# Ushio/MassiveVoxelRayTracing

Measured on AMD Instinct MI355X. Metric: Mrays/sec (primary+secondary) at 1920x1080, 64 spp, higher is better.
Workload: dtype f32; 1 GPU; xyzrgb_dragon stand-in 2048^3 SVO (procedural, pinned by tests/test_scenes.py), wavefront path trace 1920x1080, 183 steps of 16 spp rendered as 64-spp frames (frame buffer cleared + device synchronised per frame), 8 bounces + IBL shadow rays; voxels=18903401, dag_nodes=643656, triangles=1102122, parallelism=1 GPU, device= (gfx950:sramecc+:xnack-, 256 CUs)

## Files before the change

massivevoxelraytracing_amd/csrc/api.hip:

```cpp
#include <stdarg.h>
#include <stdio.h>
#include <stdlib.h>
#include <string.h>

#include <string>
#include <utility>
#include <vector>

#include "../../include/mvrt.h"
#include "launch.h"
#include "traverse_stream.h"

#define MVRT_EXPORT extern "C" __attribute__( ( visibility( "default" ) ) )

static thread_local char g_err[1024] = "";
void mvrtSetError( const char* fmt, ... )
{
	va_list ap;
	va_start( ap, fmt );
	vsnprintf( g_err, sizeof( g_err ), fmt, ap );
	va_end( ap );
}
MVRT_EXPORT const char* mvrt_last_error( void ) { return g_err; }

// ... 1083 lines not shown
	REQUIRE( pt && pt->pmj.p && tableHost, "mvrt_pt_download_pmj: call mvrt_pt_setup first" );
	MVRT_HIP( hipMemcpy( tableHost, pt->pmj.p, pt->pmj.bytes, hipMemcpyDeviceToHost ) );
	return 0;
}

MVRT_EXPORT int mvrt_pt_set_tile( mvrt_pt* pt, int tileIndex, int tileCount )
{
	REQUIRE( pt && tileCount >= 1 && tileIndex >= 0 && tileIndex < tileCount, "bad tile %d of %d", tileIndex, tileCount );
	if( pt->drain() ) return 1;
	pt->tileIndex = tileIndex;
	pt->tileCount = tileCount;
	pt->width = pt->height = 0;
	pt->fbF32.release();
	pt->releaseAovs();
	pt->releaseMoments();
	return 0;
}
MVRT_EXPORT uint64_t mvrt_pt_owned_pixels( const mvrt_pt* pt ) { return pt ? pt->ownedPixels : 0; }

static int allocWorkSlot( mvrt_pt* pt, mvrt_pt::Slot& sl )
{
	const uint64_t cap = pt->ownedPixels * MVRT_SPP_PER_STEP * pt->effectiveBatch();
	const uint64_t nBlocks = cap / 256 + 8;
	const uint64_t words = cap * ( 34 + 6 + 1 + 3 + 4 );
	const uint64_t bytes = words * 4 + cap * 3 + nBlocks * 4 + 64 * 4 + 32 * 8 + 1024 + 64 * 256;
	if( sl.work.alloc( bytes ) ) return 1;
	uint8_t* base = (uint8_t*)sl.work.p;
	uint64_t off = 0;
	auto take = [&]( uint64_t b ) {
		void* r = base + off;
		off += ( b + 255 ) & ~(uint64_t)255;
		return r;
	};
	PtBuffers& b = sl.buf;
	for( int s = 0; s < 2; s++ )
	{
		PathSet& ps = b.set[s];
		ps.task = (uint32_t*)take( cap * 4 );
		ps.org = (uint32_t*)take( cap * 4 );
		float** f[] = { &ps.rox, &ps.roy, &ps.roz, &ps.rdx, &ps.rdy, &ps.rdz, &ps.Tx, &ps.Ty, &ps.Tz, &ps.Lx, &ps.Ly, &ps.Lz, &ps.nx, &ps.ny, &ps.nz };
		for( float** q : f ) *q = (float*)take( cap * 4 );
	}
	float** d[] = { &b.sx, &b.sy, &b.sz, &b.ex, &b.ey, &b.ez, &b.hitT, &b.Lsx, &b.Lsy, &b.Lsz };
	for( float** q : d ) *q = (float*)take( cap * 4 );
	b.hitPath = (uint64_t*)take( cap * 8 );
	b.hitEPath = (uint64_t*)take( cap * 8 );
	b.hitN = (uint8_t*)take( cap );
	b.hitS = (uint8_t*)take( cap );
	b.hitE = (uint8_t*)take( cap );
	b.blockCount = (uint32_t*)take( nBlocks * 4 );
	b.liveCount = (uint32_t*)take( 64 * 4 );
	b.cursors = (unsigned long long*)take( 16 * 8 );
	b.stats = pt->statsBuf.as<unsigned long long>();
	b.cap = cap;
	b.selfDev = (const PtBuffers*)take( sizeof( PtBuffers ) );
	MVRT_HIP( hipMemset( b.liveCount, 0, 64 * 4 ) );
	MVRT_HIP( hipMemcpy( (void*)b.selfDev, &b, sizeof( PtBuffers ), hipMemcpyHostToDevice ) );
	if( pt->aovs )
	{
		if( sl.aovPart.alloc( cap / MVRT_SPP_PER_STEP * 2 * sizeof( float4 ) ) ) return 1;
	}
	else sl.aovPart.release();
	return 0;
}
static int allocWorkInner( mvrt_pt* pt );
static int forgetFrame( mvrt_pt* pt )
{
	for( mvrt_pt::Slot& sl : pt->slots )
	{
		sl.work.release();
		memset( &sl.buf, 0, sizeof( sl.buf ) );
	}
	pt->width = pt->height = 0;
	pt->fbF32.release();
	pt->fbU8.release();
	pt->releaseAovs();
	pt->releaseMoments();
	return 1;
}
static int allocWork( mvrt_pt* pt ) { return allocWorkInner( pt ) == 0 ? 0 : forgetFrame( pt ); }
static int allocWorkInner( mvrt_pt* pt )
{
	if( pt->drain() ) return 1;
	if( !pt->statsBuf.p )
	{
		if( pt->statsBuf.alloc( 64 * 8 ) ) return 1;
		MVRT_HIP( hipMemset( pt->statsBuf.p, 0, 64 * 8 ) );
	}
	if( !pt->forkEv ) MVRT_HIP( hipEventCreateWithFlags( &pt->forkEv, hipEventDisableTiming ) );
	{
		for( mvrt_pt::Slot& sl : pt->slots )
		{
			sl.work.release();
			sl.aovPart.release();
			memset( &sl.buf, 0, sizeof( sl.buf ) );
		}
		size_t freeB = 0, totalB = 0;
		MVRT_HIP( hipMemGetInfo( &freeB, &totalB ) );
		if( pt->testFreeBytes ) freeB = (size_t)pt->testFreeBytes;
		pt->batchCap = MVRT_MAX_BATCH;
		pt->depth = pt->depthWanted;
		const uint64_t budget = (uint64_t)( 0.7 * (double)freeB );
		auto need = [&]() {
			const uint64_t pathState = (uint64_t)pt->depth * pt->ownedPixels * MVRT_SPP_PER_STEP * (uint64_t)pt->effectiveBatch() * 200ull;
			const uint64_t withAovs = pt->aovs ? pathState + (uint64_t)pt->depth * pt->ownedPixels * (uint64_t)pt->effectiveBatch() * 32ull + pt->ownedPixels * 32ull : pathState;
			return pt->moments ? withAovs + pt->ownedPixels * 16ull : withAovs;
		};
		while( need() > budget && pt->effectiveBatch() > 1 ) pt->batchCap = pt->effectiveBatch() - 1;
		while( need() > budget && pt->depth > 1 ) pt->depth--;
		REQUIRE( need() <= budget, "frame of %llu owned pixels needs %.1f GB of path state, %.1f GB of HBM are free (split the frame into tiles: mvrt_pt_set_tile)",
				 (unsigned long long)pt->ownedPixels, need() / 1e9, freeB / 1e9 );
	}
	for( int i = 0; i < 4; i++ )
	{
		mvrt_pt::Slot& sl = pt->slots[i];
		if( i >= pt->depth )
		{
			sl.work.release();
			sl.aovPart.release();
			sl.trace = Workspace();
			memset( &sl.buf, 0, sizeof( sl.buf ) );
			continue;
		}
		if( allocWorkSlot( pt, sl ) ) return 1;
		if( pt->depth > 1 && !sl.stream )
		{
			const int mode = (int)mvrtKnob( "MVRT_SLOT_PRIO", 0 );
// ... 631 lines not shown
```

massivevoxelraytracing_amd/csrc/kernels_rt.hip:

```cpp
#include <stdlib.h>

#include "launch.h"
#include "traverse_stream.h"

#define WAVE 64
#define CBLOCK 256

MVRT_DI uint32_t laneId() { return __builtin_amdgcn_mbcnt_hi( ~0u, __builtin_amdgcn_mbcnt_lo( ~0u, 0u ) ); }

MVRT_DI unsigned long long waveSum( unsigned long long v )
{
	for( int o = 32; o > 0; o >>= 1 ) v += __shfl_down( v, o, WAVE );
	return v;
}

static int numCUs();

#define STREAM_WAVES_PER_CU 32

struct BatchIO
{
	const float *rox, *roy, *roz, *rdx, *rdy, *rdz;
	const uint8_t* isShadow;
	float* tOut;
	int32_t* nMajorOut;
	uint64_t* pathOut;
	uint32_t* descentsOut;
#ifdef MVRT_UTIL_STATS
	unsigned long long utilIters = 0, utilActive = 0, utilTailIters = 0, utilTailActive = 0, utilRefillClocks = 0, utilTotalClocks = 0;
	uint32_t utilMaxRayIters = 0;
#endif
	const uint64_t* originPath;
	uint32_t levels;
	MVRT_DI bool load( uint32_t i, f3* ro, f3* rd, uint32_t* hint ) const
	{
		*ro = mk3( rox[i], roy[i], roz[i] );
		*rd = mk3( rdx[i], rdy[i], rdz[i] );
		if( originPath )
		{
			const uint64_t op = originPath[i];
			if( op != ~0ull ) *hint = hintFromVoxelPath( op, levels );
		}
		return isShadow ? isShadow[i] != 0 : false;
	}
	MVRT_DI void store( uint32_t i, const StreamHit& h, bool ) const
	{
		tOut[i] = h.t;
		if( nMajorOut ) nMajorOut[i] = h.nMajor;
		if( pathOut ) pathOut[i] = h.path;
		if( descentsOut ) descentsOut[i] = h.descents;
	}
};
__global__ void __launch_bounds__( 256 ) kResolveVIndex( SvoDev svo, uint64_t n, const float* __restrict__ t, const uint64_t* __restrict__ path, const uint8_t* __restrict__ isShadow,
														  uint32_t* __restrict__ vIndexOut, uchar4* __restrict__ colorOut )
{
	for( uint64_t i = (uint64_t)blockIdx.x * 256 + threadIdx.x; i < n; i += (uint64_t)gridDim.x * 256 )
// ... 19 lines not shown
template <int FL>
__global__ void __launch_bounds__( 64, MVRT_WAVES_OF( FL ) ) kTraceBatchStream( SvoDev svo, uint64_t n, BatchIO io, TraceWorkspace ws, uint32_t chunk )
{
	__shared__ uint4 ring[MVRT_RING_OF( FL ) * 64];
	__shared__ uint32_t ringMask[FL == 0 ? 1 : ( FL == 2 ? 2 : 1 ) * MVRT_RING_OF( FL ) * 64];
	traceStream<FL>( makeTraceCore( svo ), io, n, ws.cursor, chunk, ring, ws.spill, ws.spillStride, (uint64_t)blockIdx.x * 64 + threadIdx.x, ringMask, ws.spillMask, ws.spillMask2 );
}

struct PrimaryIO
{
	SvoDev svo;
	CameraPinhole cam;
	int W, H, showVertexColor;
	uchar4* rgba;
	float* tOut;
	int32_t* nMajorOut;
	uint64_t* pathOut;
	uint32_t* descentsOut;
#ifdef MVRT_UTIL_STATS
	unsigned long long utilIters = 0, utilActive = 0, utilTailIters = 0, utilTailActive = 0, utilRefillClocks = 0, utilTotalClocks = 0;
	uint32_t utilMaxRayIters = 0;
#endif
	f3 rdKeep;
	MVRT_DI bool load( uint32_t pixelIdx, f3* ro, f3* rd, uint32_t* )
	{
		int x = (int)( pixelIdx % W );
		int y = (int)( pixelIdx / W );
		cameraShoot( cam, ro, rd, x, y, 0.5f, 0.5f, W, H );
		rdKeep = *rd;
		return false;
	}
	MVRT_DI void store( uint32_t pixelIdx, const StreamHit& r, bool ) const
	{
		uchar4 c = make_uchar4( 0, 0, 0, 255 );
		if( r.t != MVRT_MAXF )
		{
			if( !showVertexColor )
			{
				f3 hn = getHitN( r.nMajor, rdKeep );
				f3 color = ( hn + mk3( 1.0f, 1.0f, 1.0f ) ) * 0.5f;
				c = make_uchar4( (uint8_t)( 255 * color.x + 0.5f ), (uint8_t)( 255 * color.y + 0.5f ), (uint8_t)( 255 * color.z + 0.5f ), 255 );
			}
		}
		if( rgba ) rgba[pixelIdx] = c;
		if( tOut ) tOut[pixelIdx] = r.t;
		if( nMajorOut ) nMajorOut[pixelIdx] = r.nMajor;
// ... 273 lines not shown
	*step = ps / vp;
	*localPixel = ps - *step * vp;
}

MVRT_DI int dimBase( int k, int hdriEnabled, int extraSamples ) { return 2 + k * ( ( hdriEnabled ? 2 : 0 ) + 1 ) + ( k > 0 ? extraSamples : 0 ); }

__global__ void __launch_bounds__( 256 ) kPtGenerate( PtParams P )
{
	const uint64_t n = P.frame.validOwnedPixels * MVRT_SPP_PER_STEP * P.frame.nSteps;
	const PathSet& o = P.buf.set[0];
	for( uint64_t task = (uint64_t)blockIdx.x * 256 + threadIdx.x; task < n; task += (uint64_t)gridDim.x * 256 )
	{
		uint32_t step, localPixel, localSpp;
		decodeTask( P.frame, (uint32_t)task, &step, &localPixel, &localSpp );
		uint32_t pixelIdx = globalPixel( P.frame, localPixel );
		int x = pixelIdx % P.frame.width;
		int y = pixelIdx / P.frame.width;
		uint32_t spp = ( P.frame.iteration + step ) * MVRT_SPP_PER_STEP + localSpp;
		uint32_t stream = hashCombine2( 0u, pixelIdx );
		f2 camU = pmjSample2d( P.pmj, spp, 0, stream );
		f2 lensU = pmjSample2d( P.pmj, spp, 1, stream );
		f3 ro, rd;
		cameraShootThinLens( P.cams[step], &ro, &rd, x, y, camU.x, camU.y, P.frame.width, P.frame.height, lensU.x, lensU.y );
		o.task[task] = (uint32_t)task;
		o.rox[task] = ro.x;
		o.roy[task] = ro.y;
		o.roz[task] = ro.z;
		o.rdx[task] = rd.x;
		o.rdy[task] = rd.y;
		o.rdz[task] = rd.z;
	}
	for( uint64_t b = (uint64_t)blockIdx.x * 256 + threadIdx.x; b < ( n + CBLOCK - 1 ) / CBLOCK; b += (uint64_t)gridDim.x * 256 ) P.buf.blockCount[b] = 0u;
	if( blockIdx.x == 0 && threadIdx.x == 0 )
	{
		P.buf.liveCount[0] = (uint32_t)n;
		for( int k = 0; k < 16; k++ ) P.buf.cursors[k] = 0ull;
		atomicAdd( &P.buf.stats[5], (unsigned long long)n );
	}
}

template <class T>
MVRT_DI const __attribute__( ( address_space( 4 ) ) ) T* opaquePtr( const T* p )
{
	asm volatile( "" : "+s"( p ) );
	return (const __attribute__( ( address_space( 4 ) ) ) T*)p;
}

struct PtIO
{
	const PtBuffers* table;
	int setIdx;
	uint32_t n;
	int shadowKind;
	int useHint;
#ifdef MVRT_UTIL_STATS
	unsigned long long utilIters = 0, utilActive = 0, utilTailIters = 0, utilTailActive = 0, utilRefillClocks = 0, utilTotalClocks = 0;
	uint32_t utilMaxRayIters = 0;
#endif
	uint32_t dNormal, dShadow, nHits;
	MVRT_DI int kindOf( uint32_t r, uint32_t* i ) const
	{
		const uint32_t kindSlot = ( r >= n ? 1u : 0u ) + ( r >= 2u * n ? 1u : 0u );
		*i = r - ( kindSlot == 0u ? 0u : ( kindSlot == 1u ? n : 2u * n ) );
		return kindSlot == 0 ? 0 : ( kindSlot == 1 ? ( shadowKind ? 1 : 2 ) : 2 );
	}
	MVRT_DI bool load( uint32_t r, f3* ro, f3* rd, uint32_t* hint ) const
	{
		const __attribute__( ( address_space( 4 ) ) ) PtBuffers& buf = *opaquePtr( table );
		const __attribute__( ( address_space( 4 ) ) ) PathSet& in = buf.set[setIdx];
		uint32_t i;
		const int kind = kindOf( r, &i );
		*ro = mk3( in.rox[i], in.roy[i], in.roz[i] );
		if( useHint ) *hint = in.org[i];
		if( kind == 0 ) *rd = mk3( in.rdx[i], in.rdy[i], in.rdz[i] );
		else if( kind == 1 ) *rd = mk3( buf.sx[i], buf.sy[i], buf.sz[i] );
		else *rd = mk3( buf.ex[i], buf.ey[i], buf.ez[i] );
		return kind == 1;
	}
	MVRT_DI void store( uint32_t r, const StreamHit& h, bool )
	{
		const __attribute__( ( address_space( 4 ) ) ) PtBuffers& buf = *opaquePtr( table );
		uint32_t i;
		const int kind = kindOf( r, &i );
		const bool isHit = h.t != MVRT_MAXF;
		if( kind == 0 )
		{
			buf.hitT[i] = h.t;
			buf.hitPath[i] = h.path;
			buf.hitN[i] = (uint8_t)h.nMajor;
			if( isHit ) atomicAdd( &buf.blockCount[i / CBLOCK], 1u );
		}
		else if( kind == 1 )
		{
			buf.hitS[i] = isHit ? 1 : 0;
		}
		else
		{
			buf.hitE[i] = isHit ? 1 : 0;
			buf.hitEPath[i] = h.path;
		}
		dShadow += kind == 1 ? h.descents : 0u;
		dNormal += kind == 1 ? 0u : h.descents;
		nHits += ( kind != 1 && isHit ) ? 1u : 0u;
	}
};
template <int FL>
__global__ void __launch_bounds__( 64, MVRT_WAVES_OF( FL ) ) kPtTraceStream( PtParams P, TraceWorkspace ws, int stage, int setIdx, int nKinds, int shadowKind, uint32_t chunk,
																			uint32_t raysPerLane, uint32_t minWaves )
{
	__shared__ uint4 ring[MVRT_RING_OF( FL ) * 64];
	__shared__ uint32_t ringMask[FL == 0 ? 1 : ( FL == 2 ? 2 : 1 ) * MVRT_RING_OF( FL ) * 64];
	PtIO io;
	io.table = P.buf.selfDev;
	io.setIdx = setIdx;
	io.n = P.buf.liveCount[stage];
	io.shadowKind = shadowKind;
	io.useHint = ( FL == 0 && stage > 0 && P.useHints ) ? 1 : 0;
	io.dNormal = io.dShadow = io.nHits = 0;
	const uint64_t total = (uint64_t)io.n * nKinds;
	uint64_t nWaves = gridDim.x;
	if( raysPerLane )
	{
		uint64_t wantWaves = total / ( 64ull * raysPerLane ) + 1;
		if( wantWaves < minWaves ) wantWaves = minWaves;
		if( blockIdx.x >= wantWaves ) return;
		if( wantWaves < nWaves ) nWaves = wantWaves;
	}
	uint64_t c = total / ( nWaves * 4 );
	c = ( c + 63 ) / 64 * 64;
	if( c < 64 ) c = 64;
	if( c > chunk ) c = chunk;
	traceStream<FL>( makeTraceCore( P.svo ), io, total, P.buf.cursors + stage, (uint32_t)c, ring, ws.spill, ws.spillStride, (uint64_t)blockIdx.x * 64 + threadIdx.x, ringMask,
						ws.spillMask, ws.spillMask2 );
	unsigned long long dN = waveSum( (unsigned long long)io.dNormal ), dS = waveSum( (unsigned long long)io.dShadow ), nH = waveSum( (unsigned long long)io.nHits );
#ifdef MVRT_UTIL_STATS
	if( threadIdx.x == 0 )
	{
// ... 131 lines not shown
#endif
template <int WAVES>
__global__ void __launch_bounds__( CBLOCK, WAVES ) kPtShade( PtParams P, int stage, int inSet )
{
	__shared__ uint32_t waveCnt[CBLOCK / WAVE];
	const uint64_t n = P.buf.liveCount[stage];
	const PathSet& in = P.buf.set[inSet];
	const PathSet& out = P.buf.set[inSet ^ 1];
	const bool lastStage = stage >= MVRT_MAX_DEPTH;
	const uint64_t nBlocks = ( n + CBLOCK - 1 ) / CBLOCK;
	for( uint64_t vb = blockIdx.x; vb < nBlocks; vb += gridDim.x )
	{
		const uint64_t i = vb * CBLOCK + threadIdx.x;
		const bool valid = i < n;
		bool alive = false;
		uint32_t task = 0, vIndex = 0;
		uint2 attr = make_uint2( 0u, 0u );
		uint64_t hitPath = 0;
		int nMajor = 0;
		float t = MVRT_MAXF;
		f3 ro, rd, T, L;
		if( valid )
		{
			task = in.task[i];
			ro = mk3( in.rox[i], in.roy[i], in.roz[i] );
			rd = mk3( in.rdx[i], in.rdy[i], in.rdz[i] );
			t = P.buf.hitT[i];
			nMajor = P.buf.hitN[i];
			const bool hit = t != MVRT_MAXF;
			hitPath = hit ? P.buf.hitPath[i] : 0ull;
			vIndex = hit ? voxelIndexFromPath( P.svo, hitPath ) : 0u;
			if( hit ) attr = P.svo.attrs[vIndex];
			if( stage == 0 )
			{
				T = mk3( 1.0f, 1.0f, 1.0f );
				L = mk3( 0.0f, 0.0f, 0.0f );
				if( !hit )
				{
					L = L + T * hdriSampleNearest( P.hdri, rd, true );
				}
				else
				{
					L = L + T * rawReflectance( attr.y );
				}
			}
			else
			{
				T = mk3( in.Tx[i], in.Ty[i], in.Tz[i] );
				L = mk3( in.Lx[i], in.Ly[i], in.Lz[i] );
				if( P.hdriEnabled && P.buf.hitS[i] == 0 )
				{
					L = L + mk3( in.nx[i], in.ny[i], in.nz[i] );
				}
				if( stage == 1 && P.extraSamples )
				{
					if( P.buf.hitE[i] )
					{
						const uint32_t ev = voxelIndexFromPath( P.svo, P.buf.hitEPath[i] );
						f3 Le = voxelEmission( P.svo, ev, true );
						L = L + T * Le / (float)( 1 + P.extraSamples );
					}
				}
				if( hit )
				{
					f3 Le = rawReflectance( attr.y ) * P.svo.emissionScale;
					L = L + T * Le * ( stage == 1 ? 1.0f / (float)( 1 + P.extraSamples ) : 1.0f );
				}
			}
			alive = hit && !lastStage;
			if( !alive )
			{
				P.buf.Lsx[task] = L.x;
				P.buf.Lsy[task] = L.y;
				P.buf.Lsz[task] = L.z;
			}
		}
		if( lastStage ) continue;
		const uint32_t rank = blockRank( alive, waveCnt );
		const uint32_t blockOffset = P.buf.blockCount[vb];
		__syncthreads();
		if( threadIdx.x == 0 ) P.buf.blockCount[vb] = 0u;
		if( alive )
		{
			const uint64_t j = (uint64_t)blockOffset + rank;
			uint32_t step, localPixel, localSpp;
			decodeTask( P.frame, task, &step, &localPixel, &localSpp );
			const uint32_t spp = ( P.frame.iteration + step ) * MVRT_SPP_PER_STEP + localSpp;
			const uint32_t stream = hashCombine2( 0u, globalPixel( P.frame, localPixel ) );
			int dim = dimBase( stage, P.hdriEnabled, P.extraSamples );
			const f3 R = rawReflectance( attr.x );
			const f3 hitN = getHitN( nMajor, rd );
			const f3 hitP = ro + rd * t;
			f3 nee = mk3( 0.0f, 0.0f, 0.0f );
			if( P.hdriEnabled )
			{
				f2 u01 = pmjSample2d( P.pmj, spp, dim++, stream );
				f2 u23 = pmjSample2d( P.pmj, spp, dim++, stream );
				f3 sdir, emissive;
				float p;
				hdriImportanceSample( P.hdri, &sdir, &emissive, &p, hitN, u01.x, u01.y, u23.x, u23.y );
				nee = T * ( R / MVRT_PI ) * smax( dot3( hitN, sdir ), 0.0f ) * emissive / p;
				P.buf.sx[j] = sdir.x;
				P.buf.sy[j] = sdir.y;
				P.buf.sz[j] = sdir.z;
			}
			T = T * R;
			if( stage == 0 && P.extraSamples )
			{
				f2 u = pmjSample2d( P.pmj, spp, dim++, stream );
				f3 edir = sampleLambertian( u.x, u.y, hitN );
				P.buf.ex[j] = edir.x;
				P.buf.ey[j] = edir.y;
				P.buf.ez[j] = edir.z;
			}
			f2 u = pmjSample2d( P.pmj, spp, dim++, stream );
			f3 bdir = sampleLambertian( u.x, u.y, hitN );
			out.task[j] = task;
			if( P.svo.embedded ) out.org[j] = hintFromVoxelPath( hitPath, P.svo.levels );
			out.rox[j] = hitP.x;
			out.roy[j] = hitP.y;
			out.roz[j] = hitP.z;
			out.rdx[j] = bdir.x;
			out.rdy[j] = bdir.y;
			out.rdz[j] = bdir.z;
			out.Tx[j] = T.x;
			out.Ty[j] = T.y;
			out.Tz[j] = T.z;
			out.Lx[j] = L.x;
			out.Ly[j] = L.y;
			out.Lz[j] = L.z;
			out.nx[j] = nee.x;
			out.ny[j] = nee.y;
			out.nz[j] = nee.z;
		}
	}
}

__global__ void __launch_bounds__( 256 ) kPtAccumulate( PtParams P, float4* __restrict__ fb )
{
	const uint64_t n = P.frame.validOwnedPixels;
	for( uint64_t p = (uint64_t)blockIdx.x * 256 + threadIdx.x; p < n; p += (uint64_t)gridDim.x * 256 )
	{
		float4 v = fb[p];
		for( int b = 0; b < P.frame.nSteps; b++ )
		{
			const uint64_t base = ( (uint64_t)b * n + p ) * MVRT_SPP_PER_STEP;
			const float4* sx = (const float4*)( P.buf.Lsx + base );
			const float4* sy = (const float4*)( P.buf.Lsy + base );
			const float4* sz = (const float4*)( P.buf.Lsz + base );
			float ax = 0.0f, ay = 0.0f, az = 0.0f;
#pragma unroll
			for( int q = 0; q < MVRT_SPP_PER_STEP / 4; q++ )
			{
				float4 vx = sx[q], vy = sy[q], vz = sz[q];
				ax += vx.x; ax += vx.y; ax += vx.z; ax += vx.w;
				ay += vy.x; ay += vy.y; ay += vy.z; ay += vy.w;
				az += vz.x; az += vz.y; az += vz.z; az += vz.w;
			}
			v.x += ax;
			v.y += ay;
			v.z += az;
			v.w += (float)MVRT_SPP_PER_STEP;
		}
		fb[p] = v;
	}
}

struct AovRecords
{
	const float* hitT;
	const uint64_t* hitPath;
	const uint8_t* hitN;
	const float *rdx, *rdy, *rdz;
};
__global__ void __launch_bounds__( 256 ) kPtAovReduce( SvoDev svo, AovRecords r, uint64_t nPixelSteps, float4* __restrict__ partA, float4* __restrict__ partN )
{
	const uint32_t q = threadIdx.x & 3u;
	for( uint64_t ps = ( (uint64_t)blockIdx.x * 256 + threadIdx.x ) >> 2; ps < nPixelSteps; ps += (uint64_t)gridDim.x * 64 )
	{
		const uint64_t base = ps * MVRT_SPP_PER_STEP + q * 4u;
		const float4 t4 = *(const float4*)( r.hitT + base );
		const ulonglong2 p01 = *(const ulonglong2*)( r.hitPath + base ), p23 = *(const ulonglong2*)( r.hitPath + base + 2 );
		const uint32_t n4 = *(const uint32_t*)( r.hitN + base );
		const float4 dx = *(const float4*)( r.rdx + base ), dy = *(const float4*)( r.rdy + base ), dz = *(const float4*)( r.rdz + base );
		const float t[4] = { t4.x, t4.y, t4.z, t4.w };
		const uint64_t path[4] = { p01.x, p01.y, p23.x, p23.y };
		const float rx[4] = { dx.x, dx.y, dx.z, dx.w }, ry[4] = { dy.x, dy.y, dy.z, dy.w }, rz[4] = { dz.x, dz.y, dz.z, dz.w };
		uint32_t colour[4];
#pragma unroll
		for( int k = 0; k < 4; k++ ) colour[k] = t[k] != MVRT_MAXF ? svo.attrs[voxelIndexFromPath( svo, path[k] )].x : 0u;
		float acc[8] = { 0.0f, 0.0f, 0.0f, 0.0f, 0.0f, 0.0f, 0.0f, 0.0f };
#pragma unroll
		for( uint32_t turn = 0; turn < 4; turn++ )
		{
			if( q == turn )
			{
#pragma unroll
				for( int k = 0; k < 4; k++ )
				{
					if( t[k] == MVRT_MAXF ) continue;
					const f3 a = rawReflectance( colour[k] );
					const f3 n = getHitN( (int)( ( n4 >> ( 8 * k ) ) & 0xFFu ), mk3( rx[k], ry[k], rz[k] ) );
					acc[0] += a.x;
					acc[1] += a.y;
					acc[2] += a.z;
					acc[3] += 1.0f;
					acc[4] += n.x;
					acc[5] += n.y;
					acc[6] += n.z;
					acc[7] += t[k];
				}
			}
#pragma unroll
			for( int j = 0; j < 8; j++ ) acc[j] = __shfl( acc[j], (int)( ( threadIdx.x & 60u ) | turn ) );
		}
		if( q == 0 ) partA[ps] = make_float4( acc[0], acc[1], acc[2], acc[3] );
		if( q == 1 ) partN[ps] = make_float4( acc[4], acc[5], acc[6], acc[7] );
	}
}
__global__ void __launch_bounds__( 256 ) kPtAovAccumulate( uint64_t validOwnedPixels, int nSteps, const float4* __restrict__ partA, const float4* __restrict__ partN,
															 float4* __restrict__ albedo, float4* __restrict__ normalDepth )
{
	for( uint64_t p = (uint64_t)blockIdx.x * 256 + threadIdx.x; p < validOwnedPixels; p += (uint64_t)gridDim.x * 256 )
	{
		float4 a = albedo[p], n = normalDepth[p];
		for( int b = 0; b < nSteps; b++ )
		{
			const float4 pa = partA[(uint64_t)b * validOwnedPixels + p], pn = partN[(uint64_t)b * validOwnedPixels + p];
			a.x += pa.x; a.y += pa.y; a.z += pa.z; a.w += pa.w;
			n.x += pn.x; n.y += pn.y; n.z += pn.z; n.w += pn.w;
		}
		albedo[p] = a;
		normalDepth[p] = n;
	}
}

int launchPtStep( const SvoDev& svo, const TraceWorkspace& ws, const HdriDev& hdri, const float2* pmj, const CameraPinhole* cams, const PtFrame& frame,
				  const PtBuffers& buf, float4* frameBuffer, int nCUs, PtProfiler* prof, hipStream_t stream, hipEvent_t accumulateAfter, const AovBuffers* aov, float4* moments )
{
	PtParams P;
	P.svo = svo;
	P.hdri = hdri;
	P.pmj = pmj;
	for( int b = 0; b < MVRT_MAX_BATCH; b++ ) P.cams[b] = cams[b < frame.nSteps ? b : 0];
	P.frame = frame;
	P.buf = buf;
	P.hdriEnabled = ( 0.0f < hdri.scale ) ? 1 : 0;
	P.extraSamples = svo.hasEmission ? 1 : 0;
	P.useHints = frame.useHints;
	if( nCUs <= 0 ) nCUs = numCUs();

	const uint64_t nSamples = frame.validOwnedPixels * MVRT_SPP_PER_STEP * frame.nSteps;
	if( nSamples == 0 ) return 0;
	if( nSamples * 3 >= 0xFFFFFFFFull )
	{
		mvrtSetError( "batch too large: %llu samples (ray indices are 32-bit)", (unsigned long long)nSamples );
		return 1;
	}
	if( nSamples > buf.cap )
	{
		mvrtSetError( "path buffers too small: %llu samples > capacity %llu", (unsigned long long)nSamples, (unsigned long long)buf.cap );
		return 1;
	}
	if( !ws.spill )
	{
		mvrtSetError( "internal: traversal workspace missing" );
		return 1;
	}

#define PROF_BEGIN( c ) if( prof ) prof->begin( c, stream )
#define PROF_END() if( prof ) prof->end( stream )

	PROF_BEGIN( MVRT_K_OTHER );
	hipLaunchKernelGGL( kPtGenerate, dim3( persistentGrid( nSamples, 256, nCUs, 8 ) ), dim3( 256 ), 0, stream, P );
	PROF_END();

	for( int stage = 0; stage <= MVRT_MAX_DEPTH; stage++ )
	{
		const int setIdx = stage & 1;
// ... 6 lines not shown
			uint32_t smallRpl = 0, smallMinW = 0;
			{
				static const int envDiv = (int)mvrtKnob( "MVRT_TRACE_GRID_DIV", 0 );
				static const int divMaxStage = (int)mvrtKnob( "MVRT_TRACE_DIV_MAX_STAGE", 99 );
				const int div = stage > divMaxStage ? 1 : ( envDiv > 0 ? envDiv : frame.traceGridDiv );
				if( div > 1 && g > nCUs * STREAM_WAVES_PER_CU / div ) g = nCUs * STREAM_WAVES_PER_CU / div;
				static const uint32_t envRpl = (uint32_t)mvrtKnob( "MVRT_SMALL_RPL", 16 );
				static const uint32_t envMinW = (uint32_t)mvrtKnob( "MVRT_SMALL_MINW", 2048 );
				smallRpl = envRpl;
				smallMinW = envMinW;
				static const int wpc = (int)mvrtKnob( "MVRT_TRACE_WAVES_PER_CU", 0 );
				if( wpc > 0 && g > nCUs * wpc / ( div > 1 ? div : 1 ) ) g = nCUs * wpc / ( div > 1 ? div : 1 );
			}
			if( svo.embedded )
				hipLaunchKernelGGL( kPtTraceStream<0>, dim3( g ), dim3( 64 ), 0, stream, P, ws, stage, setIdx, nKinds, shadowKind, streamChunk( nSamples * nKinds, g ), smallRpl, smallMinW );
			else if( svo.tree )
				hipLaunchKernelGGL( kPtTraceStream<2>, dim3( g ), dim3( 64 ), 0, stream, P, ws, stage, setIdx, nKinds, shadowKind, streamChunk( nSamples * nKinds, g ), smallRpl, smallMinW );
			else
				hipLaunchKernelGGL( kPtTraceStream<1>, dim3( g ), dim3( 64 ), 0, stream, P, ws, stage, setIdx, nKinds, shadowKind, streamChunk( nSamples * nKinds, g ), smallRpl, smallMinW );
		}
		PROF_END();
		if( aov && stage == 0 )
		{
			const AovRecords rec = { buf.hitT, buf.hitPath, buf.hitN, buf.set[0].rdx, buf.set[0].rdy, buf.set[0].rdz };
			const uint64_t nPixelSteps = frame.validOwnedPixels * frame.nSteps;
			PROF_BEGIN( MVRT_K_OTHER );
			hipLaunchKernelGGL( kPtAovReduce, dim3( persistentGrid( nPixelSteps * 4, 256, nCUs, 8 ) ), dim3( 256 ), 0, stream, svo, rec, nPixelSteps, aov->partA, aov->partN );
			PROF_END();
		}
		PROF_BEGIN( MVRT_K_OTHER );
		static const int scanThreads = (int)mvrtKnob( "MVRT_SCAN_THREADS", 256 );
		if( scanThreads == 1024 )
			hipLaunchKernelGGL( kScanBlockCounts<1024>, dim3( 1 ), dim3( 1024 ), 0, stream, buf.blockCount, (uint64_t)0, (const uint32_t*)( buf.liveCount + stage ),
								stage < MVRT_MAX_DEPTH ? buf.liveCount + stage + 1 : (uint32_t*)nullptr, buf.stats, nKinds, shadowKind );
		else
			hipLaunchKernelGGL( kScanBlockCounts<256>, dim3( 1 ), dim3( 256 ), 0, stream, buf.blockCount, (uint64_t)0, (const uint32_t*)( buf.liveCount + stage ),
								stage < MVRT_MAX_DEPTH ? buf.liveCount + stage + 1 : (uint32_t*)nullptr, buf.stats, nKinds, shadowKind );
		PROF_END();
		PROF_BEGIN( MVRT_K_SHADE );
		{
			static const int dense = (int)mvrtKnob( "MVRT_SHADE8_STAGES", 3 );
			static const int bpc8 = (int)mvrtKnob( "MVRT_SHADE_BPC8", 8 ), bpc5 = (int)mvrtKnob( "MVRT_SHADE_BPC5", 5 );
			if( ( dense >> stage ) & 1 )
				hipLaunchKernelGGL( kPtShade<8>, dim3( persistentGrid( nSamples, CBLOCK, nCUs, bpc8 ) ), dim3( CBLOCK ), 0, stream, P, stage, setIdx );
			else
				hipLaunchKernelGGL( kPtShade<MVRT_SHADE_WAVES>, dim3( persistentGrid( nSamples, CBLOCK, nCUs, bpc5 ) ), dim3( CBLOCK ), 0, stream, P, stage, setIdx );
		}
		PROF_END();
		if( buf.dbgTasks && stage < MVRT_MAX_DEPTH )
			MVRT_HIP( hipMemcpyAsync( buf.dbgTasks + (uint64_t)stage * buf.cap, buf.set[setIdx ^ 1].task, nSamples * 4, hipMemcpyDeviceToDevice, stream ) );
	}
	if( accumulateAfter ) MVRT_HIP( hipStreamWaitEvent( stream, accumulateAfter, 0 ) );
	PROF_BEGIN( MVRT_K_OTHER );
	hipLaunchKernelGGL( kPtAccumulate, dim3( persistentGrid( frame.validOwnedPixels, 256, nCUs, 8 ) ), dim3( 256 ), 0, stream, P, frameBuffer );
	PROF_END();
	if( aov )
	{
		PROF_BEGIN( MVRT_K_OTHER );
		hipLaunchKernelGGL( kPtAovAccumulate, dim3( persistentGrid( frame.validOwnedPixels, 256, nCUs, 8 ) ), dim3( 256 ), 0, stream, frame.validOwnedPixels, frame.nSteps, aov->partA,
							aov->partN, aov->albedo, aov->normalDepth );
		PROF_END();
	}
	if( moments )
	{
		PROF_BEGIN( MVRT_K_OTHER );
		const int rc = launchPtMoments( buf, frame.validOwnedPixels, frame.nSteps, moments, nCUs, stream );
		PROF_END();
		if( rc ) return rc;
	}
	MVRT_HIP( hipGetLastError() );
	return 0;
}
```

massivevoxelraytracing_amd/csrc/launch.h:

```cpp
#pragma once
#include "devbuf.h"
#include "mvrt_common.h"

struct PathSet
{
	uint32_t* task;
	uint32_t* org;
	float *rox, *roy, *roz;
	float *rdx, *rdy, *rdz;
	float *Tx, *Ty, *Tz;
	float *Lx, *Ly, *Lz;
	float *nx, *ny, *nz;
};
struct PtBuffers
{
	PathSet set[2];
	float *sx, *sy, *sz;
	float *ex, *ey, *ez;
	float* hitT;
	uint8_t* hitN;
	uint8_t* hitS;
	uint8_t* hitE;
	uint64_t* hitPath;
	uint64_t* hitEPath;
	float *Lsx, *Lsy, *Lsz;
	uint32_t* blockCount;
	uint32_t* liveCount;
	unsigned long long* cursors;
	unsigned long long* stats;
	uint64_t cap;
	uint32_t* dbgTasks;
	const PtBuffers* selfDev;
};

struct PtFrame
{
	int width, height;
	int tileIndex, tileCount;
	uint64_t ownedPixels;
	uint64_t validOwnedPixels;
	int iteration;
	int nSteps;
	int traceGridDiv;
	int useHints;
};
#define MVRT_MAX_BATCH 8

struct TraceWorkspace
{
	uint4* spill;
	uint64_t spillStride;
	unsigned long long* cursor;
	uint64_t* paths;
	uint64_t pathCap;
	uint32_t* spillMask;
	uint32_t* spillMask2;
// ... 91 lines not shown
```

massivevoxelraytracing_amd/csrc/traverse_stream.h:

```cpp
#pragma once
#include "mvrt_common.h"

#ifndef MVRT_RING_EMBED
#define MVRT_RING_EMBED 8
#endif
#ifndef MVRT_RING_TREE
#define MVRT_RING_TREE 8
#endif
#define MVRT_RING_OF( FL ) ( ( FL ) == 0 ? MVRT_RING_EMBED : ( ( FL ) == 2 ? MVRT_RING_TREE : 4 ) )
#ifndef MVRT_REFILL_MIN_EMBED
#define MVRT_REFILL_MIN_EMBED 28
#endif
#ifndef MVRT_REFILL_MIN_TREE
#define MVRT_REFILL_MIN_TREE 12
#endif
#ifndef MVRT_REFILL_MIN_OTHER
#define MVRT_REFILL_MIN_OTHER 20
#endif
#define MVRT_REFILL_MIN_OF( FL ) ( ( FL ) == 0 ? MVRT_REFILL_MIN_EMBED : ( ( FL ) == 2 ? MVRT_REFILL_MIN_TREE : MVRT_REFILL_MIN_OTHER ) )

#define MVRT_NO_HINT 0xFFFFFFFFu
#ifndef MVRT_HINT_MAX
#define MVRT_HINT_MAX 7u
#endif
// ... 333 lines not shown
			h->nMajor = ( S == tx0 ) ? 1 : ( ( S == ty0 ) ? 2 : 0 );
		}
		else if( st == 4u )
		{
			h->t = tx1;
			h->nMajor = (int)level;
		}
		h->path = h->t != MVRT_MAXF ? path : 0ull;
		h->descents = descents;
	};

#ifdef MVRT_UTIL_STATS
	uint32_t utilVis = 0;
	const unsigned long long utilT0 = clock64();
#endif
	for( ;; )
	{
#ifdef MVRT_UTIL_STATS
		const unsigned long long utilTr = clock64();
#endif
		const unsigned long long idleMask = __ballot( st != 1u );
		const uint32_t nIdle = __popcll( idleMask );
		{
			if( st >= 2u )
			{
				StreamHit h;
				finishedHit( &h );
				io.store( ray, h, isShadow );
				st = 0;
			}
			if( !exhausted )
			{
				uint32_t need = nIdle;
				const uint32_t myRank = __popcll( idleMask & ( ( 1ull << lane ) - 1ull ) );
				uint32_t given = 0;
				while( need > 0 )
				{
					if( chunkNext == chunkEnd )
					{
						unsigned long long base = 0;
						const uint32_t c = chunk;
						if( lane == 0 ) base = atomicAdd( cursor, (unsigned long long)c );
						base = (unsigned long long)(uint32_t)__builtin_amdgcn_readfirstlane( (uint32_t)base ) | ( (unsigned long long)(uint32_t)__builtin_amdgcn_readfirstlane( (uint32_t)( base >> 32 ) ) << 32 );
						if( base >= total )
						{
							exhausted = true;
							__builtin_amdgcn_s_setprio( 3 );
							break;
						}
						chunkNext = (uint32_t)base;
						chunkEnd = ( total - chunkNext ) < c ? total : chunkNext + c;
					}
					const uint32_t avail = chunkEnd - chunkNext;
					const uint32_t take = avail < need ? avail : need;
					if( st == 0u && myRank >= given && myRank < given + take )
					{
						ray = chunkNext + ( myRank - given );
						f3 ro, rd;
						uint32_t hint = MVRT_NO_HINT;
						isShadow = io.load( ray, &ro, &rd, &hint );
						float ix = 1.0f / rd.x, iy = 1.0f / rd.y, iz = 1.0f / rd.z;
						vMask = 0;
						if( ix < 0.0f )
						{
							vMask |= 1u;
							ix = -ix;
							ro.x = s.lox + s.hix - ro.x;
						}
						if( iy < 0.0f )
						{
							vMask |= 2u;
							iy = -iy;
							ro.y = s.loy + s.hiy - ro.y;
						}
						if( iz < 0.0f )
						{
// ... 91 lines not shown
								for( uint32_t L = 0; L < MVRT_HINT_MAX; L++ )
								{
									if( L < P )
									{
										if( pending & ( 1u << L ) ) *(LdsU32*)( myRing + L * 64 ) = anc[L];
										node = k == L + 1u ? anc[L + 1] : node;
									}
								}
								inLds = pending;
								level = k;
								path = k ? (uint64_t)( hint >> ( 3u * ( P - k ) ) ) : 0ull;
								descents = k;
							}
						}
					}
					given += take;
					need -= take;
					chunkNext += take;
				}
			}
			if( __ballot( st == 1u ) == 0ull )
			{
				if( !exhausted ) continue;
				if( st >= 2u )
				{
					StreamHit h;
					finishedHit( &h );
					io.store( ray, h, isShadow );
				}
#ifdef MVRT_UTIL_STATS
				io.utilMaxRayIters = utilVis > io.utilMaxRayIters ? utilVis : io.utilMaxRayIters;
				io.utilRefillClocks += clock64() - utilTr;
				io.utilTotalClocks += clock64() - utilT0;
#endif
				break;
			}
		}

#ifdef MVRT_UTIL_STATS
		io.utilRefillClocks += clock64() - utilTr;
		{
			const unsigned long long am = __ballot( st == 1u );
			if( lane == 0 )
			{
				io.utilIters++;
				io.utilActive += __popcll( am );
// ... 165 lines not shown
```

Measured before the change: 6275 Mrays/s.

## Pack path-tracer ray and hit records into float4/uint4 AoS buffers

Converts the per-path SoA ray origin/direction, task, hint and hit arrays into packed float4/uint4 records so each load or store is a single 16-byte vector access. The trace IO now reads a per-set/per-shadow-kind pointer table into scalar registers once per refill, and splits refill chunks at kind boundaries so the direction pointer and shadow flag stay wave-uniform. This removes per-ray branching over three direction arrays and cuts the number of memory transactions. In exchange it adds padding bytes (larger path state), packs the emission hit flag into path bit 63, limits octrees to 21 levels, and replaces the debug task memcpy with a kernel.

```diff
diff --git a/massivevoxelraytracing_amd/csrc/api.hip b/massivevoxelraytracing_amd/csrc/api.hip
--- a/massivevoxelraytracing_amd/csrc/api.hip
+++ b/massivevoxelraytracing_amd/csrc/api.hip
@@ -1129,8 +1129,7 @@
 {
 	const uint64_t cap = pt->ownedPixels * MVRT_SPP_PER_STEP * pt->effectiveBatch();
 	const uint64_t nBlocks = cap / 256 + 8;
-	const uint64_t words = cap * ( 34 + 6 + 1 + 3 + 4 );
-	const uint64_t bytes = words * 4 + cap * 3 + nBlocks * 4 + 64 * 4 + 32 * 8 + 1024 + 64 * 256;
+	const uint64_t bytes = cap * ( 2 * ( 32 + 36 ) + 3 * 16 + 8 + 12 + 1 ) + nBlocks * 4 + 64 * 4 + 32 * 8 + 1024 + 64 * 256;
 	if( sl.work.alloc( bytes ) ) return 1;
 	uint8_t* base = (uint8_t*)sl.work.p;
 	uint64_t off = 0;
@@ -1143,26 +1142,29 @@
 	for( int s = 0; s < 2; s++ )
 	{
 		PathSet& ps = b.set[s];
-		ps.task = (uint32_t*)take( cap * 4 );
-		ps.org = (uint32_t*)take( cap * 4 );
-		float** f[] = { &ps.rox, &ps.roy, &ps.roz, &ps.rdx, &ps.rdy, &ps.rdz, &ps.Tx, &ps.Ty, &ps.Tz, &ps.Lx, &ps.Ly, &ps.Lz, &ps.nx, &ps.ny, &ps.nz };
+		ps.org = (float4*)take( cap * 16 );
+		ps.dir = (float4*)take( cap * 16 );
+		float** f[] = { &ps.Tx, &ps.Ty, &ps.Tz, &ps.Lx, &ps.Ly, &ps.Lz, &ps.nx, &ps.ny, &ps.nz };
 		for( float** q : f ) *q = (float*)take( cap * 4 );
 	}
-	float** d[] = { &b.sx, &b.sy, &b.sz, &b.ex, &b.ey, &b.ez, &b.hitT, &b.Lsx, &b.Lsy, &b.Lsz };
+	b.sdir = (float4*)take( cap * 16 );
+	b.edir = (float4*)take( cap * 16 );
+	b.hit = (uint4*)take( cap * 16 );
+	b.hitE = (uint64_t*)take( cap * 8 );
+	float** d[] = { &b.Lsx, &b.Lsy, &b.Lsz };
 	for( float** q : d ) *q = (float*)take( cap * 4 );
-	b.hitPath = (uint64_t*)take( cap * 8 );
-	b.hitEPath = (uint64_t*)take( cap * 8 );
-	b.hitN = (uint8_t*)take( cap );
 	b.hitS = (uint8_t*)take( cap );
-	b.hitE = (uint8_t*)take( cap );
 	b.blockCount = (uint32_t*)take( nBlocks * 4 );
 	b.liveCount = (uint32_t*)take( 64 * 4 );
 	b.cursors = (unsigned long long*)take( 16 * 8 );
 	b.stats = pt->statsBuf.as<unsigned long long>();
 	b.cap = cap;
-	b.selfDev = (const PtBuffers*)take( sizeof( PtBuffers ) );
+	b.traceTab = (const PtTraceTab*)take( 4 * sizeof( PtTraceTab ) );
 	MVRT_HIP( hipMemset( b.liveCount, 0, 64 * 4 ) );
-	MVRT_HIP( hipMemcpy( (void*)b.selfDev, &b, sizeof( PtBuffers ), hipMemcpyHostToDevice ) );
+	PtTraceTab tabs[4];
+	for( int s = 0; s < 2; s++ )
+		for( int sh = 0; sh < 2; sh++ ) tabs[s * 2 + sh] = { b.set[s].org, { b.set[s].dir, sh ? b.sdir : b.edir, b.edir }, b.hit, b.hitS, b.hitE, b.blockCount };
+	MVRT_HIP( hipMemcpy( (void*)b.traceTab, tabs, sizeof( tabs ), hipMemcpyHostToDevice ) );
 	if( pt->aovs )
 	{
 		if( sl.aovPart.alloc( cap / MVRT_SPP_PER_STEP * 2 * sizeof( float4 ) ) ) return 1;
@@ -1209,7 +1211,7 @@
 		pt->depth = pt->depthWanted;
 		const uint64_t budget = (uint64_t)( 0.7 * (double)freeB );
 		auto need = [&]() {
-			const uint64_t pathState = (uint64_t)pt->depth * pt->ownedPixels * MVRT_SPP_PER_STEP * (uint64_t)pt->effectiveBatch() * 200ull;
+			const uint64_t pathState = (uint64_t)pt->depth * pt->ownedPixels * MVRT_SPP_PER_STEP * (uint64_t)pt->effectiveBatch() * 216ull;
 			const uint64_t withAovs = pt->aovs ? pathState + (uint64_t)pt->depth * pt->ownedPixels * (uint64_t)pt->effectiveBatch() * 32ull + pt->ownedPixels * 32ull : pathState;
 			return pt->moments ? withAovs + pt->ownedPixels * 16ull : withAovs;
 		};
diff --git a/massivevoxelraytracing_amd/csrc/kernels_rt.hip b/massivevoxelraytracing_amd/csrc/kernels_rt.hip
--- a/massivevoxelraytracing_amd/csrc/kernels_rt.hip
+++ b/massivevoxelraytracing_amd/csrc/kernels_rt.hip
@@ -32,6 +32,8 @@
 #endif
 	const uint64_t* originPath;
 	uint32_t levels;
+	MVRT_DI void beginRefill() const {}
+	MVRT_DI uint32_t segment( uint32_t, uint32_t end ) const { return end; }
 	MVRT_DI bool load( uint32_t i, f3* ro, f3* rd, uint32_t* hint ) const
 	{
 		*ro = mk3( rox[i], roy[i], roz[i] );
@@ -97,6 +99,8 @@
 	uint32_t utilMaxRayIters = 0;
 #endif
 	f3 rdKeep;
+	MVRT_DI void beginRefill() const {}
+	MVRT_DI uint32_t segment( uint32_t, uint32_t end ) const { return end; }
 	MVRT_DI bool load( uint32_t pixelIdx, f3* ro, f3* rd, uint32_t* )
 	{
 		int x = (int)( pixelIdx % W );
@@ -416,13 +420,8 @@
 		f2 lensU = pmjSample2d( P.pmj, spp, 1, stream );
 		f3 ro, rd;
 		cameraShootThinLens( P.cams[step], &ro, &rd, x, y, camU.x, camU.y, P.frame.width, P.frame.height, lensU.x, lensU.y );
-		o.task[task] = (uint32_t)task;
-		o.rox[task] = ro.x;
-		o.roy[task] = ro.y;
-		o.roz[task] = ro.z;
-		o.rdx[task] = rd.x;
-		o.rdy[task] = rd.y;
-		o.rdz[task] = rd.z;
+		o.org[task] = make_float4( ro.x, ro.y, ro.z, 0.0f );
+		o.dir[task] = make_float4( rd.x, rd.y, rd.z, mvrt_u2f( (uint32_t)task ) );
 	}
 	for( uint64_t b = (uint64_t)blockIdx.x * 256 + threadIdx.x; b < ( n + CBLOCK - 1 ) / CBLOCK; b += (uint64_t)gridDim.x * 256 ) P.buf.blockCount[b] = 0u;
 	if( blockIdx.x == 0 && threadIdx.x == 0 )
@@ -433,17 +432,12 @@
 	}
 }
 
-template <class T>
-MVRT_DI const __attribute__( ( address_space( 4 ) ) ) T* opaquePtr( const T* p )
-{
-	asm volatile( "" : "+s"( p ) );
-	return (const __attribute__( ( address_space( 4 ) ) ) T*)p;
-}
-
+#define MVRT_GLOBAL __attribute__( ( address_space( 1 ) ) )
+typedef float f4v __attribute__( ( ext_vector_type( 4 ) ) );
+typedef uint32_t u2v __attribute__( ( ext_vector_type( 2 ) ) );
 struct PtIO
 {
-	const PtBuffers* table;
-	int setIdx;
+	const PtTraceTab* table;
 	uint32_t n;
 	int shadowKind;
 	int useHint;
@@ -452,46 +446,76 @@
 	uint32_t utilMaxRayIters = 0;
 #endif
 	uint32_t dNormal, dShadow, nHits;
-	MVRT_DI int kindOf( uint32_t r, uint32_t* i ) const
+	const MVRT_GLOBAL f4v* tOrg;
+	const MVRT_GLOBAL f4v* tDir0;
+	const MVRT_GLOBAL f4v* tDir1;
+	const MVRT_GLOBAL f4v* tDir2;
+	MVRT_GLOBAL u4v* tHit;
+	MVRT_GLOBAL uint8_t* tHitS;
+	MVRT_GLOBAL u2v* tHitE;
+	MVRT_GLOBAL uint32_t* tBlockCount;
+	const MVRT_GLOBAL f4v* segDir;
+	uint32_t segBase;
+	bool segShadow;
+	MVRT_DI void beginRefill()
+	{
+		const PtTraceTab* p = table;
+		asm volatile( "" : "+s"( p ) );
+		const __attribute__( ( address_space( 4 ) ) ) PtTraceTab& t = *(const __attribute__( ( address_space( 4 ) ) ) PtTraceTab*)p;
+		uint64_t a = (uint64_t)t.org, b = (uint64_t)t.dir[0], c = (uint64_t)t.dir[1], d = (uint64_t)t.dir[2], e = (uint64_t)t.hit, f = (uint64_t)t.hitS, g = (uint64_t)t.hitE,
+				 h = (uint64_t)t.blockCount;
+		asm volatile( "" : "+s"( a ), "+s"( b ), "+s"( c ), "+s"( d ), "+s"( e ), "+s"( f ), "+s"( g ), "+s"( h ) );
+		tOrg = (const MVRT_GLOBAL f4v*)a;
+		tDir0 = (const MVRT_GLOBAL f4v*)b;
+		tDir1 = (const MVRT_GLOBAL f4v*)c;
+		tDir2 = (const MVRT_GLOBAL f4v*)d;
+		tHit = (MVRT_GLOBAL u4v*)e;
+		tHitS = (MVRT_GLOBAL uint8_t*)f;
+		tHitE = (MVRT_GLOBAL u2v*)g;
+		tBlockCount = (MVRT_GLOBAL uint32_t*)h;
+	}
+	MVRT_DI uint32_t segment( uint32_t first, uint32_t end )
+	{
+		const uint32_t n2 = n + n;
+		const bool k1 = first >= n, k2 = first >= n2;
+		segBase = k2 ? n2 : ( k1 ? n : 0u );
+		uint64_t d0 = (uint64_t)tDir0, d1 = (uint64_t)tDir1, d2 = (uint64_t)tDir2;
+		asm( "" : "+s"( d0 ), "+s"( d1 ), "+s"( d2 ) );
+		segDir = (const MVRT_GLOBAL f4v*)( k2 ? d2 : ( k1 ? d1 : d0 ) );
+		segShadow = shadowKind != 0 && k1 && !k2;
+		const uint32_t bound = k2 ? 0xFFFFFFFFu : ( k1 ? n2 : n );
+		return end < bound ? end : bound;
+	}
+	MVRT_DI bool load( uint32_t r, f3* ro, f3* rd, uint32_t* hint ) const
+	{
+		const uint32_t i = r - segBase;
+		const f4v o = tOrg[i], d = segDir[i];
+		*ro = mk3( o.x, o.y, o.z );
+		if( useHint ) *hint = mvrt_f2u( o.w );
+		*rd = mk3( d.x, d.y, d.z );
+		return segShadow;
+	}
+	MVRT_DI void store( uint32_t r, const StreamHit& h, bool )
 	{
 		const uint32_t kindSlot = ( r >= n ? 1u : 0u ) + ( r >= 2u * n ? 1u : 0u );
-		*i = r - ( kindSlot == 0u ? 0u : ( kindSlot == 1u ? n : 2u * n ) );
-		return kindSlot == 0 ? 0 : ( kindSlot == 1 ? ( shadowKind ? 1 : 2 ) : 2 );
-	}
-	MVRT_DI bool load( uint32_t r, f3* ro, f3* rd, uint32_t* hint ) const
-	{
-		const __attribute__( ( address_space( 4 ) ) ) PtBuffers& buf = *opaquePtr( table );
-		const __attribute__( ( address_space( 4 ) ) ) PathSet& in = buf.set[setIdx];
-		uint32_t i;
-		const int kind = kindOf( r, &i );
-		*ro = mk3( in.rox[i], in.roy[i], in.roz[i] );
-		if( useHint ) *hint = in.org[i];
-		if( kind == 0 ) *rd = mk3( in.rdx[i], in.rdy[i], in.rdz[i] );
-		else if( kind == 1 ) *rd = mk3( buf.sx[i], buf.sy[i], buf.sz[i] );
-		else *rd = mk3( buf.ex[i], buf.ey[i], buf.ez[i] );
-		return kind == 1;
-	}
-	MVRT_DI void store( uint32_t r, const StreamHit& h, bool )
-	{
-		const __attribute__( ( address_space( 4 ) ) ) PtBuffers& buf = *opaquePtr( table );
-		uint32_t i;
-		const int kind = kindOf( r, &i );
+		const uint32_t i = r - ( kindSlot == 0u ? 0u : ( kindSlot == 1u ? n : 2u * n ) );
+		const int kind = kindSlot == 0 ? 0 : ( kindSlot == 1 ? ( shadowKind ? 1 : 2 ) : 2 );
 		const bool isHit = h.t != MVRT_MAXF;
 		if( kind == 0 )
 		{
-			buf.hitT[i] = h.t;
-			buf.hitPath[i] = h.path;
-			buf.hitN[i] = (uint8_t)h.nMajor;
-			if( isHit ) atomicAdd( &buf.blockCount[i / CBLOCK], 1u );
+			const u4v rec = { mvrt_f2u( h.t ), (uint32_t)h.nMajor, (uint32_t)h.path, (uint32_t)( h.path >> 32 ) };
+			tHit[i] = rec;
+			if( isHit ) __hip_atomic_fetch_add( &tBlockCount[i / CBLOCK], 1u, __ATOMIC_RELAXED, __HIP_MEMORY_SCOPE_AGENT );
 		}
 		else if( kind == 1 )
 		{
-			buf.hitS[i] = isHit ? 1 : 0;
+			tHitS[i] = isHit ? 1 : 0;
 		}
 		else
 		{
-			buf.hitE[i] = isHit ? 1 : 0;
-			buf.hitEPath[i] = h.path;
+			const uint64_t e = h.path | ( isHit ? MVRT_HIT_E_FLAG : 0ull );
+			const u2v rec = { (uint32_t)e, (uint32_t)( e >> 32 ) };
+			tHitE[i] = rec;
 		}
 		dShadow += kind == 1 ? h.descents : 0u;
 		dNormal += kind == 1 ? 0u : h.descents;
@@ -505,8 +529,7 @@
 	__shared__ uint4 ring[MVRT_RING_OF( FL ) * 64];
 	__shared__ uint32_t ringMask[FL == 0 ? 1 : ( FL == 2 ? 2 : 1 ) * MVRT_RING_OF( FL ) * 64];
 	PtIO io;
-	io.table = P.buf.selfDev;
-	io.setIdx = setIdx;
+	io.table = P.buf.traceTab + ( setIdx * 2 + shadowKind );
 	io.n = P.buf.liveCount[stage];
 	io.shadowKind = shadowKind;
 	io.useHint = ( FL == 0 && stage > 0 && P.useHints ) ? 1 : 0;
@@ -684,13 +707,15 @@
 		f3 ro, rd, T, L;
 		if( valid )
 		{
-			task = in.task[i];
-			ro = mk3( in.rox[i], in.roy[i], in.roz[i] );
-			rd = mk3( in.rdx[i], in.rdy[i], in.rdz[i] );
-			t = P.buf.hitT[i];
-			nMajor = P.buf.hitN[i];
+			const float4 o4 = in.org[i], d4 = in.dir[i];
+			const uint4 h4 = P.buf.hit[i];
+			task = mvrt_f2u( d4.w );
+			ro = mk3( o4.x, o4.y, o4.z );
+			rd = mk3( d4.x, d4.y, d4.z );
+			t = mvrt_u2f( h4.x );
+			nMajor = (int)( h4.y & 0xFFu );
 			const bool hit = t != MVRT_MAXF;
-			hitPath = hit ? P.buf.hitPath[i] : 0ull;
+			hitPath = hit ? ( (uint64_t)h4.z | ( (uint64_t)h4.w << 32 ) ) : 0ull;
 			vIndex = hit ? voxelIndexFromPath( P.svo, hitPath ) : 0u;
 			if( hit ) attr = P.svo.attrs[vIndex];
 			if( stage == 0 )
@@ -716,9 +741,10 @@
 				}
 				if( stage == 1 && P.extraSamples )
 				{
-					if( P.buf.hitE[i] )
+					const uint64_t e = P.buf.hitE[i];
+					if( e & MVRT_HIT_E_FLAG )
 					{
-						const uint32_t ev = voxelIndexFromPath( P.svo, P.buf.hitEPath[i] );
+						const uint32_t ev = voxelIndexFromPath( P.svo, e & ~MVRT_HIT_E_FLAG );
 						f3 Le = voxelEmission( P.svo, ev, true );
 						L = L + T * Le / (float)( 1 + P.extraSamples );
 					}
@@ -762,29 +788,19 @@
 				float p;
 				hdriImportanceSample( P.hdri, &sdir, &emissive, &p, hitN, u01.x, u01.y, u23.x, u23.y );
 				nee = T * ( R / MVRT_PI ) * smax( dot3( hitN, sdir ), 0.0f ) * emissive / p;
-				P.buf.sx[j] = sdir.x;
-				P.buf.sy[j] = sdir.y;
-				P.buf.sz[j] = sdir.z;
+				P.buf.sdir[j] = make_float4( sdir.x, sdir.y, sdir.z, 0.0f );
 			}
 			T = T * R;
 			if( stage == 0 && P.extraSamples )
 			{
 				f2 u = pmjSample2d( P.pmj, spp, dim++, stream );
 				f3 edir = sampleLambertian( u.x, u.y, hitN );
-				P.buf.ex[j] = edir.x;
-				P.buf.ey[j] = edir.y;
-				P.buf.ez[j] = edir.z;
+				P.buf.edir[j] = make_float4( edir.x, edir.y, edir.z, 0.0f );
 			}
 			f2 u = pmjSample2d( P.pmj, spp, dim++, stream );
 			f3 bdir = sampleLambertian( u.x, u.y, hitN );
-			out.task[j] = task;
-			if( P.svo.embedded ) out.org[j] = hintFromVoxelPath( hitPath, P.svo.levels );
-			out.rox[j] = hitP.x;
-			out.roy[j] = hitP.y;
-			out.roz[j] = hitP.z;
-			out.rdx[j] = bdir.x;
-			out.rdy[j] = bdir.y;
-			out.rdz[j] = bdir.z;
+			out.org[j] = make_float4( hitP.x, hitP.y, hitP.z, mvrt_u2f( P.svo.embedded ? hintFromVoxelPath( hitPath, P.svo.levels ) : 0u ) );
+			out.dir[j] = make_float4( bdir.x, bdir.y, bdir.z, mvrt_u2f( task ) );
 			out.Tx[j] = T.x;
 			out.Ty[j] = T.y;
 			out.Tz[j] = T.z;
@@ -830,10 +846,8 @@
 
 struct AovRecords
 {
-	const float* hitT;
-	const uint64_t* hitPath;
-	const uint8_t* hitN;
-	const float *rdx, *rdy, *rdz;
+	const uint4* hit;
+	const float4* dir;
 };
 __global__ void __launch_bounds__( 256 ) kPtAovReduce( SvoDev svo, AovRecords r, uint64_t nPixelSteps, float4* __restrict__ partA, float4* __restrict__ partN )
 {
@@ -841,13 +855,21 @@
 	for( uint64_t ps = ( (uint64_t)blockIdx.x * 256 + threadIdx.x ) >> 2; ps < nPixelSteps; ps += (uint64_t)gridDim.x * 64 )
 	{
 		const uint64_t base = ps * MVRT_SPP_PER_STEP + q * 4u;
-		const float4 t4 = *(const float4*)( r.hitT + base );
-		const ulonglong2 p01 = *(const ulonglong2*)( r.hitPath + base ), p23 = *(const ulonglong2*)( r.hitPath + base + 2 );
-		const uint32_t n4 = *(const uint32_t*)( r.hitN + base );
-		const float4 dx = *(const float4*)( r.rdx + base ), dy = *(const float4*)( r.rdy + base ), dz = *(const float4*)( r.rdz + base );
-		const float t[4] = { t4.x, t4.y, t4.z, t4.w };
-		const uint64_t path[4] = { p01.x, p01.y, p23.x, p23.y };
-		const float rx[4] = { dx.x, dx.y, dx.z, dx.w }, ry[4] = { dy.x, dy.y, dy.z, dy.w }, rz[4] = { dz.x, dz.y, dz.z, dz.w };
+		float t[4], rx[4], ry[4], rz[4];
+		uint64_t path[4];
+		uint32_t nm[4];
+#pragma unroll
+		for( int k = 0; k < 4; k++ )
+		{
+			const uint4 h = r.hit[base + k];
+			const float4 d = r.dir[base + k];
+			t[k] = mvrt_u2f( h.x );
+			nm[k] = h.y & 0xFFu;
+			path[k] = (uint64_t)h.z | ( (uint64_t)h.w << 32 );
+			rx[k] = d.x;
+			ry[k] = d.y;
+			rz[k] = d.z;
+		}
 		uint32_t colour[4];
 #pragma unroll
 		for( int k = 0; k < 4; k++ ) colour[k] = t[k] != MVRT_MAXF ? svo.attrs[voxelIndexFromPath( svo, path[k] )].x : 0u;
@@ -862,7 +884,7 @@
 				{
 					if( t[k] == MVRT_MAXF ) continue;
 					const f3 a = rawReflectance( colour[k] );
-					const f3 n = getHitN( (int)( ( n4 >> ( 8 * k ) ) & 0xFFu ), mk3( rx[k], ry[k], rz[k] ) );
+					const f3 n = getHitN( (int)nm[k], mk3( rx[k], ry[k], rz[k] ) );
 					acc[0] += a.x;
 					acc[1] += a.y;
 					acc[2] += a.z;
@@ -897,6 +919,11 @@
 	}
 }
 
+__global__ void __launch_bounds__( 256 ) kPtCaptureTasks( const float4* __restrict__ dir, uint64_t n, uint32_t* __restrict__ out )
+{
+	for( uint64_t i = (uint64_t)blockIdx.x * 256 + threadIdx.x; i < n; i += (uint64_t)gridDim.x * 256 ) out[i] = mvrt_f2u( dir[i].w );
+}
+
 int launchPtStep( const SvoDev& svo, const TraceWorkspace& ws, const HdriDev& hdri, const float2* pmj, const CameraPinhole* cams, const PtFrame& frame,
 				  const PtBuffers& buf, float4* frameBuffer, int nCUs, PtProfiler* prof, hipStream_t stream, hipEvent_t accumulateAfter, const AovBuffers* aov, float4* moments )
 {
@@ -917,6 +944,11 @@
 	if( nSamples * 3 >= 0xFFFFFFFFull )
 	{
 		mvrtSetError( "batch too large: %llu samples (ray indices are 32-bit)", (unsigned long long)nSamples );
+		return 1;
+	}
+	if( svo.levels > 21u )
+	{
+		mvrtSetError( "octree of %u levels: the path tracer supports at most 21", (unsigned)svo.levels );
 		return 1;
 	}
 	if( nSamples > buf.cap )
@@ -969,7 +1001,7 @@
 		PROF_END();
 		if( aov && stage == 0 )
 		{
-			const AovRecords rec = { buf.hitT, buf.hitPath, buf.hitN, buf.set[0].rdx, buf.set[0].rdy, buf.set[0].rdz };
+			const AovRecords rec = { buf.hit, buf.set[0].dir };
 			const uint64_t nPixelSteps = frame.validOwnedPixels * frame.nSteps;
 			PROF_BEGIN( MVRT_K_OTHER );
 			hipLaunchKernelGGL( kPtAovReduce, dim3( persistentGrid( nPixelSteps * 4, 256, nCUs, 8 ) ), dim3( 256 ), 0, stream, svo, rec, nPixelSteps, aov->partA, aov->partN );
@@ -995,7 +1027,7 @@
 		}
 		PROF_END();
 		if( buf.dbgTasks && stage < MVRT_MAX_DEPTH )
-			MVRT_HIP( hipMemcpyAsync( buf.dbgTasks + (uint64_t)stage * buf.cap, buf.set[setIdx ^ 1].task, nSamples * 4, hipMemcpyDeviceToDevice, stream ) );
+			hipLaunchKernelGGL( kPtCaptureTasks, dim3( persistentGrid( nSamples, 256, nCUs, 8 ) ), dim3( 256 ), 0, stream, buf.set[setIdx ^ 1].dir, nSamples, buf.dbgTasks + (uint64_t)stage * buf.cap );
 	}
 	if( accumulateAfter ) MVRT_HIP( hipStreamWaitEvent( stream, accumulateAfter, 0 ) );
 	PROF_BEGIN( MVRT_K_OTHER );
diff --git a/massivevoxelraytracing_amd/csrc/launch.h b/massivevoxelraytracing_amd/csrc/launch.h
--- a/massivevoxelraytracing_amd/csrc/launch.h
+++ b/massivevoxelraytracing_amd/csrc/launch.h
@@ -4,25 +4,29 @@
 
 struct PathSet
 {
-	uint32_t* task;
-	uint32_t* org;
-	float *rox, *roy, *roz;
-	float *rdx, *rdy, *rdz;
+	float4* org;
+	float4* dir;
 	float *Tx, *Ty, *Tz;
 	float *Lx, *Ly, *Lz;
 	float *nx, *ny, *nz;
 };
+struct PtTraceTab
+{
+	const float4* org;
+	const float4* dir[3];
+	uint4* hit;
+	uint8_t* hitS;
+	uint64_t* hitE;
+	uint32_t* blockCount;
+};
 struct PtBuffers
 {
 	PathSet set[2];
-	float *sx, *sy, *sz;
-	float *ex, *ey, *ez;
-	float* hitT;
-	uint8_t* hitN;
+	float4* sdir;
+	float4* edir;
+	uint4* hit;
 	uint8_t* hitS;
-	uint8_t* hitE;
-	uint64_t* hitPath;
-	uint64_t* hitEPath;
+	uint64_t* hitE;
 	float *Lsx, *Lsy, *Lsz;
 	uint32_t* blockCount;
 	uint32_t* liveCount;
@@ -30,8 +34,9 @@
 	unsigned long long* stats;
 	uint64_t cap;
 	uint32_t* dbgTasks;
-	const PtBuffers* selfDev;
+	const PtTraceTab* traceTab;
 };
+#define MVRT_HIT_E_FLAG ( 1ull << 63 )
 
 struct PtFrame
 {
diff --git a/massivevoxelraytracing_amd/csrc/traverse_stream.h b/massivevoxelraytracing_amd/csrc/traverse_stream.h
--- a/massivevoxelraytracing_amd/csrc/traverse_stream.h
+++ b/massivevoxelraytracing_amd/csrc/traverse_stream.h
@@ -379,6 +379,7 @@
 		const unsigned long long idleMask = __ballot( st != 1u );
 		const uint32_t nIdle = __popcll( idleMask );
 		{
+			io.beginRefill();
 			if( st >= 2u )
 			{
 				StreamHit h;
@@ -408,7 +409,7 @@
 						chunkNext = (uint32_t)base;
 						chunkEnd = ( total - chunkNext ) < c ? total : chunkNext + c;
 					}
-					const uint32_t avail = chunkEnd - chunkNext;
+					const uint32_t avail = io.segment( chunkNext, chunkEnd ) - chunkNext;
 					const uint32_t take = avail < need ? avail : need;
 					if( st == 0u && myRank >= given && myRank < given + take )
 					{
@@ -546,6 +547,7 @@
 			if( __ballot( st == 1u ) == 0ull )
 			{
 				if( !exhausted ) continue;
+				io.beginRefill();
 				if( st >= 2u )
 				{
 					StreamHit h;
```

Measured after the change: 6322 Mrays/s (median of 6 runs). No clear change (+0.7%).
